# aditya-v-kallappa/FInCFlow

Measured on AMD Instinct MI355X. Metric: inverse images/sec (+ fwd+logdet ms/img in `forward`), 3x3 conv @64x64x96, higher is better.
Workload: dtype f32

## Files before the change

### fincflow_amd/csrc/finc_abi.hip

```cpp
#include "finc_common.h"

#include <stdlib.h>
#include <string.h>

#include <atomic>
#include <mutex>
#include <utility>
#include <vector>

namespace {

thread_local char g_hip_error[256] = "no error";

std::mutex g_table_mutex;
std::vector<std::pair<int, const void *>> g_attr_done;
constexpr int MAX_DEVICES = 64;
int *g_invariant_flag[MAX_DEVICES];
volatile unsigned *g_fault_host[MAX_DEVICES];
unsigned *g_fault_dev[MAX_DEVICES];
std::vector<std::pair<int, size_t>> g_debug_tokens;

std::atomic<bool> g_fault_armed_any{false};
std::vector<const char *> g_env_seen;

// ... 98 lines not shown

int finc_fault_gate(bool arm, hipStream_t st)
{
    if (!arm && !g_fault_armed_any.load(std::memory_order_acquire)) return FINC_OK;
    int dev = 0;
    FINC_HIP_TRY(hipGetDevice(&dev));
    if (dev < 0 || dev >= MAX_DEVICES) return FINC_ERR_BAD_DIMS;
    volatile unsigned *w = g_fault_host[dev];
    if (!w && arm) {
        hipStreamCaptureStatus cs = hipStreamCaptureStatusNone;
        if (hipStreamIsCapturing(st, &cs) != hipSuccess) { (void)hipGetLastError(); cs = hipStreamCaptureStatusNone; }
        if (cs == hipStreamCaptureStatusNone) {
            std::lock_guard<std::mutex> lk(g_table_mutex);
            if (!g_fault_host[dev]) {
                unsigned *h = nullptr, *d = nullptr;
                FINC_HIP_TRY(hipHostMalloc((void **)&h, sizeof(unsigned), hipHostMallocMapped));
                *h = 0;
                int e = FINC_OK;
                if (hipError_t he = hipHostGetDevicePointer((void **)&d, h, 0); he != hipSuccess) { finc_set_hip_error(he); e = FINC_ERR_LAUNCH; }
                if (!e) e = finc_mfma_arm_fault_word(d);
                if (e) { (void)hipHostFree(h); return e; }
                g_fault_dev[dev] = d;
                g_fault_host[dev] = h;
                g_fault_armed_any.store(true, std::memory_order_release);
            }
            w = g_fault_host[dev];
        }
    }
    if (w && *w != 0) {
        strncpy(g_hip_error, "a helper-wave wait of an earlier launch on this device gave up: its output is not valid (finc_clear_fault() resets)",
                sizeof(g_hip_error) - 1);
        return FINC_ERR_LAUNCH;
    }
    return FINC_OK;
}

template <typename T>
static int canonicalize(const T *w_stored, T *w_canon, int G, int Cq, int KH, int KW, unsigned orient, finc_stream_t stream)
{
    if (!w_stored || !w_canon) return FINC_ERR_NULL_POINTER;
    if (int e = check_shape(1, G, Cq, 1, 1, KH, KW)) return e;
    if (w_stored == w_canon) return FINC_ERR_BAD_DIMS;
    const int total = G * Cq * Cq * KH * KW;
    int blocks = (total + 255) / 256;
    if (blocks > 1024) blocks = 1024;
    hipLaunchKernelGGL(canonicalize_kernel<T>, dim3(blocks), dim3(256), 0, (hipStream_t)stream, w_stored, w_canon, G,
                       Cq, KH, KW, orient);
    FINC_CHECK_LAUNCH();
    return FINC_OK;
}

extern "C" {

int finc_version(void) { return 105; }

unsigned finc_build_flags(void)
{
    return FINC_BUILD_FLAGS | finc_build_flags_mfma() | finc_build_flags_split() | finc_build_flags_chain() | finc_build_flags_f64() | finc_build_flags_conv() | finc_build_flags_gradw() | finc_build_flags_wino4m() |
           finc_build_flags_mix() | finc_build_flags_generic() | finc_build_flags_wino() | finc_build_flags_big() | finc_build_flags_probe() | finc_build_flags_wino5() | finc_build_flags_stream();
}

int finc_fault_pending(void)
{
    int dev = 0;
    if (hipGetDevice(&dev) != hipSuccess || dev < 0 || dev >= MAX_DEVICES) return 0;
    volatile unsigned *w = g_fault_host[dev];
    return (w && *w != 0) ? 1 : 0;
}

int finc_runtime_switches(char *h_buf, size_t n)
{
    std::lock_guard<std::mutex> lk(g_table_mutex);
    size_t used = 0;
    int count = 0;
    auto put = [&](const char *t) {
        const size_t l = strlen(t);
        if (h_buf && used + l + 2 < n) {
            if (used) h_buf[used++] = ',';
            memcpy(h_buf + used, t, l);
            used += l;
        }
        ++count;
    };
    for (const char *name : g_env_seen) put(name);
    if (finc_wino_form_override() != 0) put("forward_form_override");
    if (h_buf && n) h_buf[used < n ? used : n - 1] = 0;
    return count;
}

int finc_clear_fault(void)
{
    int dev = 0;
    FINC_HIP_TRY(hipGetDevice(&dev));
    if (dev < 0 || dev >= MAX_DEVICES) return FINC_ERR_BAD_DIMS;
    if (g_fault_host[dev]) *g_fault_host[dev] = 0;
    return FINC_OK;
}

const char *finc_status_string(int status)
{
    switch (status) {
    case FINC_OK: return "ok";
    case FINC_ERR_NULL_POINTER: return "null pointer argument";
    case FINC_ERR_BAD_DIMS: return "bad dimensions";
    case FINC_ERR_UNSUPPORTED: return "requested algorithm does not support this shape";
    case FINC_ERR_WORKSPACE: return "workspace missing or too small";
    case FINC_ERR_LAUNCH: return "HIP call failed";
// ... 511 lines not shown
```

### fincflow_amd/csrc/finc_mfma.hip

```cpp
#include "finc_common.h"
#include "finc_tile.h"

#include <stdlib.h>

#include <mutex>
#include <type_traits>
#include <utility>
#include <vector>

namespace {

typedef float v4f __attribute__((ext_vector_type(4)));
typedef unsigned v2u __attribute__((ext_vector_type(2)));
typedef unsigned v4u __attribute__((ext_vector_type(4)));

template <int CQP_, int KH_, int KW_, int NW_ = 1>
struct Cfg {
    static constexpr int CQP = CQP_, KH = KH_, KW = KW_, NW = NW_;
    static constexpr int MTB = CQP / 16;
    static constexpr int NSM = (CQP % 16) / 4;
    static constexpr int MT = MTB + NSM;
    static constexpr int NKZT = CQP / 4;
    static constexpr int NKDT = CQP / 4;
    static_assert(NW == 1 || (NKZT % NW == 0 && NKDT % NW == 0), "K-split must divide the k-steps and the output registers");
    static constexpr int NKZ = NKZT / NW;
    static constexpr int NKD = NKDT / NW;
    static constexpr int NK = NKD;
    static constexpr int NTAP = KH * KW;
    static constexpr int NFRAG = (NKZ + (NTAP - 1) * NKD) * MT;
    static constexpr int NFRAGT = (NKZT + (NTAP - 1) * NKDT) * MT;
    static constexpr int NPACK = NFRAGT + 8 * MT;
    static constexpr int ZSLOTS = 12, XSLOTS = 8;
    static constexpr int ZRING = NKZ * ZSLOTS * 64;
    static constexpr int XRING = NKD * XSLOTS * 64;
    static constexpr bool XALIAS = NW == 2;
    static constexpr bool PAIR = finc_pair_bank(CQP, KH, KW) && NW == 1;
    static constexpr int NPAIR = 2 * NKDT;
    static constexpr int XCH = (NW > 1 && !XALIAS) ? NW * NW * NKD * 64 : 0;
};

__host__ __device__ inline int chan_d(int MTB, int j, int q)
{
    if (j < 4 * MTB) return 16 * (j >> 2) + 4 * q + (j & 3);
    return 16 * MTB + 4 * (j - 4 * MTB) + q;
}

template <int N>
__device__ inline float row_shr(float old, float src)
{
    return __builtin_bit_cast(float, __builtin_amdgcn_update_dpp(__builtin_bit_cast(int, old),
                                                                 __builtin_bit_cast(int, src), 0x110 + N, 0xf, 0xf,
                                                                 false));
}

template <int A>
struct ShiftOp {
    template <int NK>
    static __device__ inline void apply(float (&dst)[NK], const float (&fifo)[NK], const float (&src)[NK])
    {
#pragma unroll
        for (int j = 0; j < NK; ++j) dst[j] = row_shr<A>(fifo[j], src[j]);
    }
};

template <class C>
__device__ inline void pack_d(const v4f (&acc)[C::MT], float (&xpk)[C::NKDT])
{
#pragma unroll
    for (int mt = 0; mt < C::MTB; ++mt) {
        xpk[4 * mt + 0] = acc[mt].x;
        xpk[4 * mt + 1] = acc[mt].y;
        xpk[4 * mt + 2] = acc[mt].z;
        xpk[4 * mt + 3] = acc[mt].w;
    }
#pragma unroll
    for (int sb = 0; sb < C::NSM; ++sb) xpk[4 * C::MTB + sb] = finc_block_reduce(acc[C::MTB + sb]);
}

template <int KH, int KW>
struct BTaps {
    static constexpr int count()
    {
        int n = 0;
        for (int a = 0; a < KH; ++a)
            for (int b = 0; b < KW; ++b) n += (a + b >= 2);
        return n;
    }
    static constexpr int a_of(int i)
    {
        for (int a = 0; a < KH; ++a)
            for (int b = 0; b < KW; ++b)
                if (a + b >= 2 && i-- == 0) return a;
        return 0;
    }
    static constexpr int b_of(int i)
    {
        for (int a = 0; a < KH; ++a)
            for (int b = 0; b < KW; ++b)
// ... 74 lines not shown
        __builtin_amdgcn_make_buffer_rsrc((void *)(in + (size_t)bg_in * CQ * HW), 0, (int)slab_bytes, 0x00020000);
    const __amdgpu_buffer_rsrc_t rout =
        __builtin_amdgcn_make_buffer_rsrc((void *)(out + (size_t)bg_out * CQ * HW), 0, (int)slab_bytes, 0x00020000);
    const int D = W - P + 1;
    const int fifo_n = D * SS;
    const int wave_lds = C::ZRING + C::XRING + fifo_n + SS + 64;
    float *const lds_p = lds + prob * (C::XCH + NW * wave_lds);
    float *xch = lds_p;
    float *zring = lds_p + C::XCH + wv * wave_lds;
    float *xring = zring + C::ZRING;
    auto zcell = [](int qq, int rr) {
        const int lo = ((rr >> 2) ^ ((0x3200 >> (4 * (rr & 3))) & 3)) | ((qq & 1) << 2);
        return lo | (((rr & 3) | ((qq >> 1) << 2)) << 3);
    };
    float *fifo = xring + C::XRING;
    const int trash = fifo_n + lane;
    const unsigned flag_a = (unsigned)(uintptr_t)(lds + 4 * wave_lds + 4 * prob);
    auto flag_set = [flag_a](auto word_c, int v) {
        constexpr int WORD = decltype(word_c)::value;
        (void)flag_a;
#ifdef FINC_HLP_INJECT_TIMEOUT
        if (WORD == 1 && v >= 8) return;
#endif
        if constexpr (HLP) asm volatile("ds_write_b32 %0, %1 offset:%2" ::"v"(flag_a), "v"(v), "n"(4 * WORD) : "memory");
    };
    auto flag_peek = [flag_a](auto word_c, int &reg) {
        constexpr int WORD = decltype(word_c)::value;
        (void)flag_a;
        if constexpr (HLP) asm volatile("ds_read_b32 %0, %1 offset:%2" : "=v"(reg) : "v"(flag_a), "n"(4 * WORD) : "memory");
    };
    auto flag_wait = [flag_a](auto word_c, int target) {
        constexpr int WORD = decltype(word_c)::value;
#ifndef FINC_HLP_NOWAIT
#define FINC_HLP_NOWAIT 0
#endif
        if constexpr (HLP && !((FINC_HLP_NOWAIT >> WORD) & 1)) {
            int budget = 1 << FINC_HLP_BUDGET_LOG2;
            for (; budget > 0; --budget) {
                int v;
                asm volatile("ds_read_b32 %0, %1 offset:%2\n\ts_waitcnt lgkmcnt(0)" : "=v"(v) : "v"(flag_a), "n"(4 * WORD) : "memory");
                if (__builtin_amdgcn_readfirstlane(v) >= target) break;
                __builtin_amdgcn_s_sleep(2);
            }
            if (budget == 0 && (threadIdx.x & 63) == 0) {
                atomicAdd(&finc_hlp_timeouts, 1u);
                if (finc_fault_word) __hip_atomic_store(finc_fault_word, 1u, __ATOMIC_RELAXED, __HIP_MEMORY_SCOPE_SYSTEM);
            }
        }
    };

    constexpr int NSMALL = (NFRAG / MT) * C::NSM, NSR = (NSMALL + 3) / 4;
    float af[NFRAG];
    float afs[NSR > 0 ? NSR : 1];
    float afp[C::PAIR ? C::NPAIR : 1];
    static_assert(!C::PAIR || ((NKZ * C::NSM) % 4 == 0 && (NK * C::NSM) % 4 == 0),
                  "a packed block register must not straddle a paired and an unpaired tap");
    auto small_paired = [](int sfr) {
        const int tapi = sfr < NKZ * C::NSM ? 0 : 1 + (sfr - NKZ * C::NSM) / (NK * (C::NSM > 0 ? C::NSM : 1));
        return C::PAIR && tapi >= 1 && tapi <= 4;
    };
    if (!helper) {
        const float *pk = packed + (size_t)g * C::NPACK * 64 + lane;
        auto gindex = [&](int f) {
            if (f < NKZ * MT) return (wv * NKZ + f / MT) * MT + f % MT;
            const int ff = f - NKZ * MT;
            return C::NKZT * MT + ((ff / (MT * NKD)) * C::NKDT + wv * NKD + (ff / MT) % NKD) * MT + ff % MT;
        };
#pragma unroll
        for (int f = 0; f < NFRAG; ++f) {
            if (f % MT >= C::MTB) continue;
            if (ZPRE && f < NKZ * MT) { af[f] = 0.f; continue; }
            if (NW == 1 && f < NKZ * MT && finc_zterm_is_zero(C::MTB, f / MT, f % MT)) { af[f] = 0.f; continue; }
            af[f] = pk[gindex(f) * 64];
        }
        const int quad = (lane & 15) >> 2;
#pragma unroll
        for (int r = 0; r < NSR; ++r) {
            if (small_paired(4 * r)) { afs[r] = 0.f; continue; }
            int gi = 0;
#pragma unroll
            for (int a = 3; a >= 0; --a) {
                const int sfr = 4 * r + a < NSMALL ? 4 * r + a : NSMALL - 1;
                constexpr int NSMD = C::NSM > 0 ? C::NSM : 1;
                const int f = (sfr / NSMD) * MT + C::MTB + sfr % NSMD;
                const int ga = gindex(f);
                gi = (a == 3 || quad == a) ? ga : gi;
            }
            afs[r] = pk[gi * 64];
        }
#pragma unroll
        for (int f = 0; f < NFRAG; ++f) {
            if (f % MT >= C::MTB) continue;
            if (ZPRE && f < NKZ * MT) continue;
            if (NW == 1 && f < NKZ * MT && finc_zterm_is_zero(C::MTB, f / MT, f % MT)) continue;
            asm volatile("" : "+a"(af[f]));
        }
#pragma unroll
        for (int r = 0; r < NSR; ++r) {
            if (small_paired(4 * r)) continue;
            asm volatile("" : "+a"(afs[r]));
        }
        if constexpr (C::PAIR) {
            const float *pp = packed + finc_pair_offset(G, C::NPACK, C::NPAIR, g, 0) + lane;
#pragma unroll
            for (int f = 0; f < C::NPAIR; ++f) afp[f] = pp[f * 64];
#pragma unroll
            for (int f = 0; f < C::NPAIR; ++f) asm volatile("" : "+a"(afp[f]));
        }
    }
    auto mma = [&](v4f &acc_, int f, float b) {
        const int mt = f % MT;
        if (mt < C::MTB) acc_ = __builtin_amdgcn_mfma_f32_16x16x4f32(af[f], b, acc_, 0, 0, 0);
        else {
            const int sfr = (f / MT) * C::NSM + (mt - C::MTB);
            finc_mma_small(acc_, afs[sfr >> 2], b, sfr & 3);
        }
    };
    v4f bias[MT];
    {
        const float *pb = packed + ((size_t)g * C::NPACK + C::NFRAGT + (wv == 0 ? 0 : 4 * MT)) * 64 + lane;
#pragma unroll
        for (int mt = 0; mt < MT; ++mt)
            bias[mt] = (v4f){pb[(4 * mt + 0) * 64], pb[(4 * mt + 1) * 64], pb[(4 * mt + 2) * 64], pb[(4 * mt + 3) * 64]};
    }
    for (int i = lane; i < fifo_n + SS + 64; i += 64) fifo[i] = 0.f;

    const int fl4 = -((p + 3) >> 2);
    const int k0 = fw ? 3 : 0, k1 = fw ? 2 : 1, k2 = fw ? 1 : 2, k3 = fw ? 0 : 3;
    const unsigned lane_t = 4u * (unsigned)q * HW * 4u, lane_b = (unsigned)q * HW * 4u;
    unsigned cmask[NKD];
#pragma unroll
    for (int j = 0; j < NKD; ++j) cmask[j] = chan_d(C::MTB, wv * NKD + j, q) < CQ ? 0u : OFF_BAD_CHANNEL;
    const unsigned zlast = (4 * (wv * NKZ + NKZ - 1) + q) < CQ ? 0u : OFF_BAD_CHANNEL;
    unsigned zpad[NW > 1 ? NKZ : 1];
    if constexpr (NW > 1) {
#pragma unroll
        for (int j = 0; j < NKZ; ++j) zpad[j] = (4 * (wv * NKZ + j) + q) < CQ ? 0u : OFF_BAD_CHANNEL;
    }
    auto zmark = [&](int j) { return NW > 1 ? zpad[j] : (j == NKZ - 1 ? zlast : 0u); };
    const int rowstep = (fh ? -P : P) * W * 4;
    const int dirw = fw ? -1 : 1;

    constexpr unsigned long long PARTNER = 0xCBAFED8943276501ull;
    const int cls = ((p + 3) >> 2) & 1;
    const int part = (int)((PARTNER >> (4 * p)) & 15);
    int srvrow[2], srvhalf[2];
#pragma unroll
    for (int wp = 0; wp < 2; ++wp) {
        const bool own = cls == wp || p >= P;
        srvrow[wp] = own ? p : part;
        srvhalf[wp] = own ? 0 : 1;
    }
    int lcolS[2], lrowS[2], loffS[2], lslotS[2], ldst[2];
    int scolS[2], srowS[2], soffS[2];
#pragma unroll
    for (int wp = 0; wp < 2; ++wp) {
        const int R = srvrow[wp], h = srvhalf[wp];
        const int f = -((R + 3) >> 2);
        lcolS[wp] = 4 * ((wp ? -3 : -4) + 4 + f);
        lrowS[wp] = R;
// ... 439 lines not shown
                s64_part(IC<0>{}, IC<VMS>{}, w, IC<1>{});
                flag_wait(IC<0>{}, w);
                sec_sread(IC<1>{}, w + 1);
                s64_part(IC<0>{}, IC<VMS>{}, 0, IC<2>{});
                sec_swrite(IC<1>{}, 0, NKD);
                flag_wait(IC<3>{}, w + 1);
                s64_part(IC<1>{}, IC<VMS>{}, w + 1, IC<1>{});
                flag_wait(IC<0>{}, w + 1);
                sec_sread(IC<0>{}, w + 2);
                s64_part(IC<1>{}, IC<VMS>{}, 0, IC<2>{});
                sec_swrite(IC<0>{}, 0, NKD);
            }
            return;
        }
    }

    if constexpr (HLP) {
    } else if constexpr (SEC) {
        sec_event(IC<0>{});
        sec_event(IC<1>{});
        sec_event(IC<0>{});
        s64_event(IC<0>{}, IC<0>{});
        s64_event(IC<1>{}, IC<0>{});
        s64_event(IC<0>{}, IC<0>{});
    } else {
        io_issue(0, NKZ, true);
        io_land();
        io_issue(0, NKZ, true);
    }

    int nslot = ((-3 - p) % 12 + 12) % 12;
    const float *zrd = zring + (nslot >> 2) * 256 + 4 * zcell(q, p) + (fw ? 3 - (nslot & 3) : (nslot & 3));
    int zstep[4];
#pragma unroll
    for (int ph = 0; ph < 4; ++ph) zstep[ph] = (((ph + 2 - p) & 3) == 0) ? 256 - 3 * dirw : dirw;
    int tp1 = -3;
    int tm = -3;
    int xwin = 256 + lane;
    int win = 0;
    int peek_b = -1, peek_b2 = 0;

    {
        constexpr int FZ = 0;
        constexpr int FT = NKZ * MT;
        using BT = BTaps<KH, KW>;
        constexpr int NCH = BT::count();
        v4f acc[MT];
#pragma unroll
        for (int mt = 0; mt < MT; ++mt) acc[mt] = (v4f){0.f, 0.f, 0.f, 0.f};
        float zqc[C::NSM > 0 ? C::NSM : 1], zqn[C::NSM > 0 ? C::NSM : 1];
#pragma unroll
        for (int sb = 0; sb < (C::NSM > 0 ? C::NSM : 1); ++sb) zqc[sb] = zqn[sb] = 0.f;
        v4f accp = (v4f){0.f, 0.f, 0.f, 0.f};

        auto phase_a = [&](auto pha_c, int j0, int j1) {
            constexpr int PHA = decltype(pha_c)::value;
#pragma unroll
            for (int j = j0; j < j1; ++j)
#pragma unroll
                for (int mt = 0; mt < (C::PAIR ? C::MTB : MT); ++mt) {
                    if constexpr (KW > 1)
                        mma(acc[mt], FT + ((0 * KW + 1 - 1) * NK + j) * MT + mt, ROT ? Q[0][(PHA + 3) & 3][j] : R[0][1][j]);
                    if constexpr (KH > 1)
                        mma(acc[mt], FT + ((1 * KW + 0 - 1) * NK + j) * MT + mt, ROT ? Q[1][(PHA + 3) & 3][j] : R[1][0][j]);
                }
            if constexpr (C::PAIR) {
#pragma unroll
                for (int j = j0; j < j1; ++j) {
                    accp = __builtin_amdgcn_mfma_f32_16x16x4f32(afp[j], Q[0][(PHA + 3) & 3][j], accp, 0, 0, 0);
                    accp = __builtin_amdgcn_mfma_f32_16x16x4f32(afp[NK + j], Q[1][(PHA + 3) & 3][j], accp, 0, 0, 0);
                }
            }
        };

#ifdef FINC_STAMP
        unsigned stamp_acc[40];
#pragma unroll
        for (int i = 0; i < 40; ++i) stamp_acc[i] = 0u;
        unsigned long long stamp_prev = 0;
        bool stamp_on = false;
#endif
        auto step = [&](auto ph_c, auto wp_c) {
            constexpr int PH = decltype(ph_c)::value;
            FINC_STAMP_AT(9);
            const bool any_wrap = tm >= 0 && tm < P;
            const bool any_idle = tp1 < P - 1;
            float zraw[NKZ], zv[NKZ], xpk[NKD];
            float xown[NKD];
            v4f accn[MT];
            if constexpr (HLP && PH == 0) {
                asm volatile("s_waitcnt lgkmcnt(0)" ::: "memory");
                if (__builtin_expect(__builtin_amdgcn_readfirstlane(peek_b) < win, 0)) { FINC_COLD(); FINC_HLP_LATE(0); flag_wait(IC<1>{}, win); }
            }
            if constexpr (HLP && PH == 1) flag_peek(IC<2>{}, peek_b2);
            if constexpr (C::PAIR) {
                float rs[C::NSM];
#pragma unroll
                for (int sb = 0; sb < C::NSM; ++sb) {
                    rs[sb] = finc_block_reduce(acc[C::MTB + sb]);
                    if constexpr (ZPRE) rs[sb] += zqc[sb];
                }
                const float c0 = accp.z, c1 = accp.w;
                accp = (v4f){c0 + rs[0], c1 + rs[1], 0.f, 0.f};
            }

#pragma unroll
            for (int j = 0; j < NKZ; ++j) zraw[j] = FINC_ABLATE >= 3 ? af[j] : zrd[j * C::ZSLOTS * 64];
            if constexpr (!ROT) {
#pragma unroll
                for (int a = 0; a < KH; ++a) {
#pragma unroll
                    for (int b = KW - 1; b >= 1; --b) {
                        if (a + b >= 2) {
#pragma unroll
                            for (int j = 0; j < NK; ++j) R[a][b][j] = R[a][b - 1][j];
                        }
                    }
                    if (a >= 2) {
#pragma unroll
                        for (int j = 0; j < NK; ++j) R[a][0][j] = DL[a][a - 2][j];
                    }
                }
                if (__builtin_expect(any_wrap, 0)) {
                    FINC_COLD();
                    const bool wrapn = p == tm;
#pragma unroll
                    for (int a = 0; a < KH; ++a)
#pragma unroll
                        for (int b = 1; b < KW; ++b) {
                            if (a + b >= 2) {
#pragma unroll
                                for (int j = 0; j < NK; ++j) R[a][b][j] = wrapn ? 0.f : R[a][b][j];
                            }
                        }
                }
            }
            phase_a(ph_c, 0, NK / 2);
            if constexpr (HLP && PH == 3) flag_set(IC<3>{}, win + 1);
            FINC_SB();
#pragma unroll
            for (int j = 0; j < NKZ; ++j) zv[j] = zraw[j];
            if (__builtin_expect(any_idle, 0)) {
                FINC_COLD();
                const bool started = p <= tp1;
#pragma unroll
                for (int j = 0; j < NKZ; ++j) zv[j] = started ? zv[j] : 0.f;
            }
            phase_a(ph_c, NK / 2, NK);
            FINC_STAMP_AT(0);
            if constexpr (ROT) {
                if (__builtin_expect(any_wrap, 0)) {
                    FINC_COLD();
                    const bool wrapn = p == tm;
#pragma unroll
                    for (int a = 0; a < KH; ++a)
#pragma unroll
                        for (int b = 1; b < KW; ++b) {
                            if (a + b >= 2) {
#pragma unroll
                                for (int j = 0; j < NK; ++j)
                                    Q[a][(PH + 9 - a - b) & 3][j] = wrapn ? 0.f : Q[a][(PH + 9 - a - b) & 3][j];
                            }
                        }
                }
            }
            FINC_SB();
            if constexpr (ZPRE) {
#pragma unroll
                for (int mt = 0; mt < C::MTB; ++mt) accn[mt] = (v4f){zv[4 * mt], zv[4 * mt + 1], zv[4 * mt + 2], zv[4 * mt + 3]};
#pragma unroll
                for (int sb = 0; sb < C::NSM; ++sb) {
                    accn[C::MTB + sb] = (v4f){0.f, 0.f, 0.f, 0.f};
                    zqn[sb] = zv[4 * C::MTB + sb];
                }
            } else if (__builtin_expect(any_idle, 0)) {
                FINC_COLD();
                const bool started = p <= tp1;
#pragma unroll
                for (int mt = 0; mt < MT; ++mt) {
                    const float b0 = bias[mt].x, b1 = bias[mt].y, b2 = bias[mt].z, b3 = bias[mt].w;
                    accn[mt] = (v4f){started ? b0 : 0.f, started ? b1 : 0.f, started ? b2 : 0.f, started ? b3 : 0.f};
                    mma(accn[mt], FZ + mt, zv[0]);
                }
            } else {
#pragma unroll
                for (int mt = 0; mt < MT; ++mt) {
                    accn[mt] = bias[mt];
                    mma(accn[mt], FZ + mt, zv[0]);
                }
            }
#pragma unroll
            for (int j = 1; j < NKZ; ++j)
#pragma unroll
                for (int mt = 0; mt < MT; ++mt) {
                    if (ZPRE) continue;
                    if (NW == 1 && finc_zterm_is_zero(C::MTB, j, mt)) continue;
                    mma(accn[mt], FZ + j * MT + mt, zv[j]);
                }
            FINC_STAMP_AT(1);
            if constexpr (NW > 1) {
                float vv[C::NKDT];
                pack_d<C>(acc, vv);
#pragma unroll
                for (int d = 0; d < C::NKDT; ++d) {
                    const int dst = d / NKD;
                    if (dst != wv) {
                        if constexpr (C::XALIAS)
                            (lds_p + dst * wave_lds + C::ZRING)[(d % NKD) * C::XSLOTS * 64 + PH * 64 + xwin] = vv[d];
                        else
                            xch[((dst * NW + wv) * NKD + d % NKD) * 64 + lane] = vv[d];
                    }
                    else xown[d % NKD] = vv[d];
                }
                FINC_SB();
                __syncthreads();
            }
            FINC_SB();

            auto post1 = [&]() {
                if constexpr (FINC_ABLATE >= 2 && NW == 1) {
                    pack_d<C>(acc, xpk);
#pragma unroll
                    for (int j = 0; j < NKD; ++j) asm volatile("" ::"v"(xpk[j]));
                    return;
                }
                if constexpr (C::PAIR) {
#pragma unroll
                    for (int mt = 0; mt < C::MTB; ++mt) {
                        xpk[4 * mt + 0] = acc[mt].x;
                        xpk[4 * mt + 1] = acc[mt].y;
                        xpk[4 * mt + 2] = acc[mt].z;
                        xpk[4 * mt + 3] = acc[mt].w;
                    }
                    xpk[4 * C::MTB + 0] = accp.x;
                    xpk[4 * C::MTB + 1] = accp.y;
                    if (__builtin_expect(any_wrap, 0)) {
                        FINC_COLD();
                        const bool wrapn = p == tm;
                        const float c0 = accp.z, c1 = accp.w;
                        accp.z = wrapn ? 0.f : c0;
                        accp.w = wrapn ? 0.f : c1;
                    }
                } else if constexpr (NW == 1) {
                    pack_d<C>(acc, xpk);
                    if constexpr (ZPRE) {
#pragma unroll
                        for (int sb = 0; sb < C::NSM; ++sb) xpk[4 * C::MTB + sb] += zqc[sb];
                    }
                } else {
#pragma unroll
                    for (int j = 0; j < NKD; ++j) {
                        float sum = xown[j];
#pragma unroll
                        for (int src = 0; src < NW; ++src)
                            if (src != wv)
                                sum += C::XALIAS ? xring[j * C::XSLOTS * 64 + PH * 64 + xwin]
                                                 : xch[((wv * NW + src) * NKD + j) * 64 + lane];
                        xpk[j] = sum;
                    }
                }
#pragma unroll
                for (int j = 0; j < NKD; ++j) xring[j * C::XSLOTS * 64 + PH * 64 + xwin] = xpk[j];
                if constexpr (KH > 1) {
                    fifo_push(xpk);
                    fifo_pop_all();
                }
                if constexpr (KW > 1) {
                    if (__builtin_expect(any_wrap, 0)) {
                        FINC_COLD();
                        const bool wrapn = p == tm;
#pragma unroll
                        for (int j = 0; j < NK; ++j) (ROT ? Q[0][PH][j] : R[0][1][j]) = wrapn ? 0.f : xpk[j];
                    } else {
#pragma unroll
                        for (int j = 0; j < NK; ++j) (ROT ? Q[0][PH][j] : R[0][1][j]) = xpk[j];
                    }
                }
            };
            auto post2 = [&]() { if constexpr (FINC_ABLATE < 2) shift_all(xpk, ph_c); };

            auto chunk = [&](auto ci_c) {
                constexpr int CI = decltype(ci_c)::value;
                constexpr int a = BT::a_of(CI), b = BT::b_of(CI);
#pragma unroll
                for (int j = 0; j < NK; ++j)
#pragma unroll
                    for (int mt = 0; mt < ((C::PAIR && a + b == 2 && a < 2) ? C::MTB : MT); ++mt)
                        mma(accn[mt], FT + ((a * KW + b - 1) * NK + j) * MT + mt, ROT ? Q[a][(PH + 9 - a - b) & 3][j] : R[a][b][j]);
                if constexpr (CI == 0) {
                    if constexpr (HLP && PH == 1) {
                        asm volatile("s_waitcnt lgkmcnt(0)" ::: "memory");
                        if (__builtin_expect(__builtin_amdgcn_readfirstlane(peek_b2) < win + 1, 0)) { FINC_COLD(); FINC_HLP_LATE(1); flag_wait(IC<2>{}, win + 1); }
                    }
                    post1();
                    if constexpr (HLP && PH == 3) flag_set(IC<0>{}, win + 1);
                }
                if constexpr (!HLP && CI == (NCH > 1 ? 1 : 0)) io_phase(ph_c, wp_c);
                if constexpr (CI == (NCH > 2 ? 2 : NCH - 1)) {
                    post2();
                    if constexpr (HLP && PH == 3) flag_peek(IC<1>{}, peek_b);
                }
                FINC_SB();
                if constexpr (CI < 6) FINC_STAMP_AT(2 + CI);
            };
            if constexpr (NCH == 0) {
                post1();
                io_phase(ph_c, wp_c);
                post2();
                FINC_SB();
            } else {
                [&]<int... I>(std::integer_sequence<int, I...>) { (chunk(IC<I>{}), ...); }
                (std::make_integer_sequence<int, NCH>{});
            }
#pragma unroll
            for (int mt = 0; mt < MT; ++mt) acc[mt] = accn[mt];
            if constexpr (ZPRE) {
#pragma unroll
                for (int sb = 0; sb < C::NSM; ++sb) zqc[sb] = zqn[sb];
            }
            if constexpr (NW > 1) __syncthreads();
            ++tp1;
            ++tm; if (tm == W) tm = 0;
            ++nslot; zrd += zstep[PH];
            if (nslot == 12) { nslot = 0; zrd -= 12 * 64; }
            if constexpr (PH == 3) { xwin ^= 256; ++win; }
            fifo_advance();
            FINC_STAMP_AT(8);
        };

        if constexpr (HLP) {
        } else if constexpr (SEC) {
            sec_sread(IC<1>{});
            sec_swrite(IC<1>{}, 0, NKD);
            sec_event(IC<1>{});
            s64_event(IC<1>{}, IC<0>{});
        } else {
            io_sread();
            io_swrite(0, NKD);
            io_land();
            io_issue(0, NKZ, true);
        }
// ... 112 lines not shown
        }
        packed[((size_t)g * npack + f) * 64 + lane] = (float)v;
    }
    for (int e = threadIdx.x; e < npair * 64; e += blockDim.x) {
        const int lane = e & 63, f = e >> 6;
        int row, j, q, a, b;
        finc_pair_elem(MTB, NKD, f, lane, &row, &j, &q, &a, &b);
        const int col = chan_d(MTB, j, q);
        double v = 0.0;
        if (row < Cq && col < Cq) {
            const int widx = (KH - 1 - a) * KW + (KW - 1 - b);
            for (int k = 0; k <= row; ++k) v -= Linv[row * Cq + k] * (double)wg[((size_t)k * Cq + col) * KK + widx];
        }
        packed[finc_pair_offset(gridDim.x, npack, npair, g, f) + lane] = (float)v;
    }
    for (int e = threadIdx.x; e < 8 * MT * 64; e += blockDim.x) {
        const int lane = e & 63, f = e >> 6;
        const int q = lane >> 4, mt = (f % (4 * MT)) >> 2, r = f & 3;
        const int row = mt < MTB ? 16 * mt + 4 * q + r : (q == 0 ? 16 * MTB + 4 * (mt - MTB) + r : Cq);
        double v = 0.0;
        if (f < 4 * MT && shift && row < Cq)
            for (int k = 0; k <= row; ++k) v += Linv[row * Cq + k] * (double)shift[g * Cq + k];
        packed[((size_t)g * npack + nfrag + f) * 64 + lane] = (float)v;
    }
}

typedef void (*wave_fn)(const float *, const float *, float *, int, int, int, int, int, int, unsigned);

struct Inst {
    int cqp, kh, kw;
    wave_fn fn;
    wave_fn fn_sec;
    wave_fn fn_s64;
    wave_fn fn_hlp;
    wave_fn fn_zpre;
    int nkz, nkd, nk, mt, nfrag, mtb;
    int nw, wnkz, wnkd;
    int npw;
    int max_problems;
};

template <int CQP, int KH, int KW, int NW = 1, int NPW = 1, int MAXP = 0>
constexpr Inst make_inst()
{
    using C = Cfg<CQP, KH, KW, NW>;
    constexpr int zskip = [] {
        int n = 0;
        for (int j = 0; j < C::NKZ; ++j)
            for (int mt = 0; mt < C::MTB; ++mt) n += finc_zterm_is_zero(C::MTB, j, mt) ? 1 : 0;
        return n;
    }();
    constexpr bool one = NW == 1 && NPW == 1;
    constexpr int pinned = (C::NFRAG / C::MT) * C::MTB - zskip + ((C::NFRAG / C::MT) * C::NSM + 3) / 4;
    static_assert(!C::PAIR || C::NPAIR == C::NK * C::NSM, "paired fragments must replace as many packed block registers");
    constexpr int mode = !one ? 0 : (pinned + 8 * C::NKZ + 8 * C::NKD <= 256) ? 3 : (pinned + 8 * C::NKD <= 256) ? 1 : 0;
    wave_fn f64 = nullptr, fhl = nullptr, fzp = nullptr;
    if constexpr (mode != 0) f64 = finc_wave_kernel<CQP, KH, KW, true, NW, NPW, mode>;
#ifndef FINC_HLP_MODE
#define FINC_HLP_MODE 1
#endif
    constexpr bool hlp_fits = 16 * C::NKZ + 4 * C::NKD <= 124 && 12 * C::NKD + 48 <= 124 && pinned <= 124 && (KH - 1 + KW) < 6;
    if constexpr (mode == 3 && FINC_HLP_MODE && hlp_fits) {
        fhl = finc_wave_kernel<CQP, KH, KW, true, NW, NPW, 3, 1>;
        fzp = finc_wave_kernel<CQP, KH, KW, true, NW, NPW, 3, 1, true>;
    }
    return Inst{CQP, KH, KW, finc_wave_kernel<CQP, KH, KW, false, NW, NPW>, finc_wave_kernel<CQP, KH, KW, true, NW, NPW>, f64, fhl, fzp,
                C::NKZT, C::NKDT, C::NK, C::MT, C::NFRAGT, C::MTB, NW, C::NKZ, C::NKD, NPW, MAXP};
}

#ifdef FINC_ONLY_C3
const Inst g_insts[] = {make_inst<24, 3, 3, 2, 2, 512>(), make_inst<24, 3, 3>(), make_inst<12, 3, 3>()};
#else
const Inst g_insts[] = {
    make_inst<4, 3, 3>(),  make_inst<8, 3, 3>(),  make_inst<12, 3, 3>(), make_inst<16, 3, 3>(),
    make_inst<20, 3, 3>(),
    make_inst<24, 3, 3, 2, 2, 512>(), make_inst<24, 3, 3>(), make_inst<28, 3, 3>(),
    make_inst<32, 3, 3, 2, 2>(), make_inst<32, 3, 3>(),
    make_inst<40, 3, 3, 2, 2>(), make_inst<40, 3, 3, 2>(), make_inst<48, 3, 3, 4>(), make_inst<64, 3, 3, 4>(),
    make_inst<4, 2, 2>(),  make_inst<8, 2, 2>(),  make_inst<12, 2, 2>(), make_inst<16, 2, 2>(), make_inst<24, 2, 2>(),
    make_inst<32, 2, 2, 2, 2>(), make_inst<32, 2, 2>(),
    make_inst<4, 5, 5>(),  make_inst<8, 5, 5>(),  make_inst<12, 5, 5>(), make_inst<16, 5, 5>(),
    make_inst<24, 5, 5, 2>(), make_inst<32, 5, 5, 4>(), make_inst<48, 5, 5, 4>(),
    make_inst<4, 3, 5>(),  make_inst<8, 3, 5>(),  make_inst<16, 3, 5>(),
    make_inst<4, 2, 3>(),  make_inst<8, 2, 3>(),  make_inst<16, 2, 3>(),
};
#endif

size_t lds_bytes(const Inst &i, int W, int P);

bool finc_no_hlp()
{
    static const bool off = [] { const char *e = finc_env("FINC_NO_HLP"); return e && e[0] == '1'; }();
    return off;
}

bool finc_no_s64()
{
    static const bool off = [] { const char *e = finc_env("FINC_NO_S64"); return e && e[0] == '1'; }();
    return off;
}

int padded_cq(int Cq, int KH, int KW)
{
    int best = 0;
    for (const Inst &i : g_insts)
        if (i.cqp >= Cq && i.kh == KH && i.kw == KW && (best == 0 || i.cqp < best)) best = i.cqp;
    if (best && best - Cq > 3) {
// ... 40 lines not shown
{
    const size_t D = (size_t)(W - P + 1);
    const size_t ss = (size_t)i.nk * 4 * (i.kh - 1);
    const size_t per_wave = (size_t)i.wnkz * 12 * 64 + (size_t)i.wnkd * 8 * 64 + D * ss + ss + 64;
    const size_t xch = i.nw > 2 ? (size_t)i.nw * i.nw * i.wnkd * 64 : 0;
    return sizeof(float) * (size_t)i.npw * (xch + (size_t)i.nw * per_wave);
}

}

#ifdef FINC_STAMP
extern "C" int finc_debug_stamps(unsigned long long *host_out, int n)
{
    return (int)hipMemcpyFromSymbol(host_out, HIP_SYMBOL(finc_stamp_buf), sizeof(unsigned long long) * (size_t)n);
}
#endif

int finc_mfma_arm_fault_word(unsigned *device_ptr_to_host_word)
{
    FINC_HIP_TRY(hipMemcpyToSymbol(HIP_SYMBOL(finc_fault_word), &device_ptr_to_host_word, sizeof(device_ptr_to_host_word)));
    return FINC_OK;
}

int finc_mfma_hlp_timeouts(unsigned *count)
{
    FINC_HIP_TRY(hipMemcpyFromSymbol(count, HIP_SYMBOL(finc_hlp_timeouts), sizeof(unsigned)));
    return FINC_OK;
}

static bool stream_bank(int Cq, int KH, int KW)
{
    return !finc_big_bank(Cq, KH, KW) && padded_cq(Cq, KH, KW) == 0 && finc_stream_bank_ok(Cq, KH, KW);
}

static const Inst *bank_inst(int Cq, int KH, int KW)
{
    const int cqp = padded_cq(Cq, KH, KW);
    for (const Inst &i : g_insts)
        if (cqp && i.cqp == cqp && i.kh == KH && i.kw == KW) return &i;
    return nullptr;
}
static const Inst *borrowed_inst(int Cq, int KH, int KW)
{
    const int b = borrowed_cqp(padded_cq(Cq, KH, KW), KH, KW);
    if (b)
        for (const Inst &k : g_insts)
            if (k.cqp == b && k.kh == KH && k.kw == KW && k.nw == 2 && k.npw == 2) return &k;
    return nullptr;
}
static int pair_frags(const Inst *i)
{
    if (!finc_pair_bank(i->cqp, i->kh, i->kw)) return 0;
    for (const Inst &k : g_insts)
        if (k.cqp == i->cqp && k.kh == i->kh && k.kw == i->kw && k.nw == 1) return 2 * i->nkd;
    return 0;
}
static size_t bank_bytes(const Inst *i, int G) { return i ? (size_t)(i->nfrag + 8 * i->mt + pair_frags(i)) * 64 * sizeof(float) * (size_t)G : 0; }
static size_t wave_bank_bytes(int G, int Cq, int KH, int KW)
{
    return bank_bytes(bank_inst(Cq, KH, KW), G) + bank_bytes(borrowed_inst(Cq, KH, KW), G);
}

enum InvForm {
    INV_NONE,
    INV_TABLE,
    INV_SPLIT,
    INV_BIG,
    INV_WIDE,
    INV_STREAM,
};

struct InvPlan {
    InvForm form = INV_NONE;
    const Inst *inst = nullptr;
    int io = 0;
    wave_fn fn = nullptr;
    size_t lds = 0;
    int grid = 0, block = 0;
    size_t bank_offset = 0;
    int tail_images = 0;
    bool zpre = false;
    bool affine = false;
    bool align16 = true;
    FincSplitPlan split{};
};

static InvForm inverse_form(int Cq, int H, int W, int KH, int KW)
{
    if (finc_big_bank(Cq, KH, KW)) return finc_big_supported(Cq, H, W, KH, KW) ? INV_BIG : INV_NONE;
    if (stream_bank(Cq, KH, KW)) return finc_stream_supported(Cq, H, W, KH, KW, true) ? INV_STREAM : INV_NONE;
    if (W % 4 != 0 || W < 4 || H < 1) return INV_NONE;
    const int P = W < 16 ? W : 16;
    if (P < KH - 1) return INV_NONE;
    if (!find_inst(padded_cq(Cq, KH, KW), KH, KW, -1, W))
        return finc_big_wide_bank(Cq, KH, KW) && finc_big_supported(Cq, H, W, KH, KW) ? INV_WIDE : INV_NONE;
    if ((size_t)Cq * H * W * 4 >= ((size_t)1 << 30)) return INV_NONE;
    return INV_TABLE;
}

static InvPlan inverse_plan(const FincShape &s)
{
    InvPlan p;
    p.form = inverse_form(s.Cq, s.H, s.W, s.KH, s.KW);
    if (p.form == INV_NONE) return p;
    p.affine = p.form != INV_BIG && p.form != INV_WIDE;
    if (p.form == INV_WIDE) p.bank_offset = wave_bank_bytes(s.G, s.Cq, s.KH, s.KW);
    if (p.form == INV_BIG || p.form == INV_WIDE) return p;
// ... 206 lines not shown
```

### fincflow_amd/csrc/finc_tile.h

```cpp
#pragma once
#include <stddef.h>

typedef float finc_v4f __attribute__((ext_vector_type(4)));
typedef unsigned finc_v2u __attribute__((ext_vector_type(2)));

template <int MTB>
__device__ inline void finc_mma(finc_v4f &acc, int mt, float a, float b)
{
    if (mt < MTB) acc = __builtin_amdgcn_mfma_f32_16x16x4f32(a, b, acc, 0, 0, 0);
    else acc = __builtin_amdgcn_mfma_f32_4x4x1f32(a, b, acc, 0, 0, 0);
}

__device__ inline void finc_mma_small(finc_v4f &acc, float a4, float b, int abid)
{
    switch (abid & 3) {
    case 0: acc = __builtin_amdgcn_mfma_f32_4x4x1f32(a4, b, acc, 2, 0, 0); break;
    case 1: acc = __builtin_amdgcn_mfma_f32_4x4x1f32(a4, b, acc, 2, 1, 0); break;
    case 2: acc = __builtin_amdgcn_mfma_f32_4x4x1f32(a4, b, acc, 2, 2, 0); break;
    default: acc = __builtin_amdgcn_mfma_f32_4x4x1f32(a4, b, acc, 2, 3, 0); break;
    }
}

__device__ inline float finc_block_reduce(const finc_v4f &acc)
{
    const float r0 = acc.x, r1 = acc.y, r2 = acc.z, r3 = acc.w;
    const finc_v2u a = __builtin_amdgcn_permlane32_swap(__builtin_bit_cast(unsigned, r0), __builtin_bit_cast(unsigned, r2),
                                                        false, false);
    const finc_v2u b = __builtin_amdgcn_permlane32_swap(__builtin_bit_cast(unsigned, r1), __builtin_bit_cast(unsigned, r3),
                                                        false, false);
    const unsigned a0 = a.x, a1 = a.y, b0 = b.x, b1 = b.y;
    const float s02 = __builtin_bit_cast(float, a0) + __builtin_bit_cast(float, a1);
    const float s13 = __builtin_bit_cast(float, b0) + __builtin_bit_cast(float, b1);
    const finc_v2u c = __builtin_amdgcn_permlane16_swap(__builtin_bit_cast(unsigned, s02), __builtin_bit_cast(unsigned, s13),
                                                        false, false);
    const unsigned c0 = c.x, c1 = c.y;
    return __builtin_bit_cast(float, c0) + __builtin_bit_cast(float, c1);
}

__host__ __device__ constexpr bool finc_zterm_is_zero(int MTB, int j, int mt)
{
    return mt < MTB ? 4 * j > 16 * mt + 15 : 4 * j > 16 * MTB + 4 * (mt - MTB) + 3;
}

__host__ __device__ inline int finc_tile_row(int MTB, int mt, int i)
{
    return mt < MTB ? 16 * mt + i : 16 * MTB + 4 * (mt - MTB) + (i & 3);
}

__host__ __device__ constexpr bool finc_pair_bank(int cqp, int KH, int KW) { return KH == 3 && KW == 3 && cqp > 16 && cqp % 16 == 8; }
__host__ __device__ inline int finc_pair_row(int MTB, int i, int *partner)
{
    const int qq = i >> 2, r = i & 3;
    *partner = r >> 1;
    return 16 * MTB + 4 * (r & 1) + qq;
}
__host__ __device__ inline void finc_pair_elem(int MTB, int NKD, int f, int lane, int *row, int *j, int *q, int *a, int *b)
{
    int partner;
    const int pr = f / NKD;
    *row = finc_pair_row(MTB, lane & 15, &partner);
    *j = f % NKD;
    *q = lane >> 4;
    *a = pr == 0 ? 0 : 1;
    *b = (pr == 0 ? 1 : 0) + partner;
}
__host__ __device__ inline size_t finc_pair_offset(int G, int npack, int npair, int g, int f)
{
    return ((size_t)G * npack + (size_t)g * npair + f) * 64;
}
```

Before: 635,100.

## Extend paired-tap MFMA packing to the bottom kernel row in helper kernels

Adds a second stage of paired-fragment packing so that taps 6 and 7 (third kernel row) of the 3x3 wave kernel for odd-16 channel counts are computed with one 16x16x4 MFMA per k-step instead of separate small 4x4 block MFMAs. The carried column values go into a separate register pair and a new accumulator. The wrap test becomes a scalar sign-bit check. The new path is active only in helper (HLP) instantiations. It grows the paired weight bank from two to three fragments per k-step, which adds register and memory pressure and changes the packed layout every consumer must agree on.

```diff
diff --git a/fincflow_amd/csrc/finc_abi.hip b/fincflow_amd/csrc/finc_abi.hip
--- a/fincflow_amd/csrc/finc_abi.hip
+++ b/fincflow_amd/csrc/finc_abi.hip
@@ -174,7 +174,7 @@
 
 extern "C" {
 
-int finc_version(void) { return 105; }
+int finc_version(void) { return 106; }
 
 unsigned finc_build_flags(void)
 {
diff --git a/fincflow_amd/csrc/finc_mfma.hip b/fincflow_amd/csrc/finc_mfma.hip
--- a/fincflow_amd/csrc/finc_mfma.hip
+++ b/fincflow_amd/csrc/finc_mfma.hip
@@ -35,7 +35,8 @@
     static constexpr int XRING = NKD * XSLOTS * 64;
     static constexpr bool XALIAS = NW == 2;
     static constexpr bool PAIR = finc_pair_bank(CQP, KH, KW) && NW == 1;
-    static constexpr int NPAIR = 2 * NKDT;
+    static constexpr int NPAIR = 3 * NKDT;
+    static constexpr int NPAIR1 = 2 * NKDT;
     static constexpr int XCH = (NW > 1 && !XALIAS) ? NW * NW * NKD * 64 : 0;
 };
 
@@ -44,6 +45,9 @@
     if (j < 4 * MTB) return 16 * (j >> 2) + 4 * q + (j & 3);
     return 16 * MTB + 4 * (j - 4 * MTB) + q;
 }
+
+template <class C>
+__host__ __device__ constexpr bool finc_pair2_form(bool hlp) { return C::PAIR && hlp; }
 
 template <int N>
 __device__ inline float row_shr(float old, float src)
@@ -224,12 +228,14 @@
     constexpr int NSMALL = (NFRAG / MT) * C::NSM, NSR = (NSMALL + 3) / 4;
     float af[NFRAG];
     float afs[NSR > 0 ? NSR : 1];
-    float afp[C::PAIR ? C::NPAIR : 1];
+    constexpr bool PAIR2 = finc_pair2_form<C>(HLP);
+    constexpr int NPAIRF = PAIR2 ? C::NPAIR : C::NPAIR1;
+    float afp[C::PAIR ? NPAIRF : 1];
     static_assert(!C::PAIR || ((NKZ * C::NSM) % 4 == 0 && (NK * C::NSM) % 4 == 0),
                   "a packed block register must not straddle a paired and an unpaired tap");
     auto small_paired = [](int sfr) {
         const int tapi = sfr < NKZ * C::NSM ? 0 : 1 + (sfr - NKZ * C::NSM) / (NK * (C::NSM > 0 ? C::NSM : 1));
-        return C::PAIR && tapi >= 1 && tapi <= 4;
+        return C::PAIR && ((tapi >= 1 && tapi <= 4) || (PAIR2 && (tapi == 6 || tapi == 7)));
     };
     if (!helper) {
         const float *pk = packed + (size_t)g * C::NPACK * 64 + lane;
@@ -275,9 +281,9 @@
         if constexpr (C::PAIR) {
             const float *pp = packed + finc_pair_offset(G, C::NPACK, C::NPAIR, g, 0) + lane;
 #pragma unroll
-            for (int f = 0; f < C::NPAIR; ++f) afp[f] = pp[f * 64];
-#pragma unroll
-            for (int f = 0; f < C::NPAIR; ++f) asm volatile("" : "+a"(afp[f]));
+            for (int f = 0; f < NPAIRF; ++f) afp[f] = pp[f * 64];
+#pragma unroll
+            for (int f = 0; f < NPAIRF; ++f) asm volatile("" : "+a"(afp[f]));
         }
     }
     auto mma = [&](v4f &acc_, int f, float b) {
@@ -823,6 +829,8 @@
 #pragma unroll
         for (int sb = 0; sb < (C::NSM > 0 ? C::NSM : 1); ++sb) zqc[sb] = zqn[sb] = 0.f;
         v4f accp = (v4f){0.f, 0.f, 0.f, 0.f};
+        v4f accq = (v4f){0.f, 0.f, 0.f, 0.f};
+        float cy[2] = {0.f, 0.f};
 
         auto phase_a = [&](auto pha_c, int j0, int j1) {
             constexpr int PHA = decltype(pha_c)::value;
@@ -854,7 +862,17 @@
         auto step = [&](auto ph_c, auto wp_c) {
             constexpr int PH = decltype(ph_c)::value;
             FINC_STAMP_AT(9);
-            const bool any_wrap = tm >= 0 && tm < P;
+            std::conditional_t<C::PAIR, int, bool> wrap_state;
+            if constexpr (C::PAIR) wrap_state = (tm - P) & ~tm;
+            else wrap_state = tm >= 0 && tm < P;
+            auto any_wrap = [&]() -> bool {
+                if constexpr (C::PAIR) {
+                    asm volatile("" : "+s"(wrap_state));
+                    return wrap_state < 0;
+                } else {
+                    return wrap_state;
+                }
+            };
             const bool any_idle = tp1 < P - 1;
             float zraw[NKZ], zv[NKZ], xpk[NKD];
             float xown[NKD];
@@ -871,8 +889,14 @@
                     rs[sb] = finc_block_reduce(acc[C::MTB + sb]);
                     if constexpr (ZPRE) rs[sb] += zqc[sb];
                 }
-                const float c0 = accp.z, c1 = accp.w;
-                accp = (v4f){c0 + rs[0], c1 + rs[1], 0.f, 0.f};
+                if constexpr (PAIR2) {
+                    accp = accq;
+                    accp.x += cy[0] + rs[0];
+                    accp.y += cy[1] + rs[1];
+                } else {
+                    const float c0 = accp.z, c1 = accp.w;
+                    accp = (v4f){c0 + rs[0], c1 + rs[1], 0.f, 0.f};
+                }
             }
 
 #pragma unroll
@@ -892,7 +916,7 @@
                         for (int j = 0; j < NK; ++j) R[a][0][j] = DL[a][a - 2][j];
                     }
                 }
-                if (__builtin_expect(any_wrap, 0)) {
+                if (__builtin_expect(any_wrap(), 0)) {
                     FINC_COLD();
                     const bool wrapn = p == tm;
 #pragma unroll
@@ -920,7 +944,7 @@
             phase_a(ph_c, NK / 2, NK);
             FINC_STAMP_AT(0);
             if constexpr (ROT) {
-                if (__builtin_expect(any_wrap, 0)) {
+                if (__builtin_expect(any_wrap(), 0)) {
                     FINC_COLD();
                     const bool wrapn = p == tm;
 #pragma unroll
@@ -1005,12 +1029,21 @@
                     }
                     xpk[4 * C::MTB + 0] = accp.x;
                     xpk[4 * C::MTB + 1] = accp.y;
-                    if (__builtin_expect(any_wrap, 0)) {
+                    if constexpr (PAIR2) {
+                        cy[0] = accp.z;
+                        cy[1] = accp.w;
+                    }
+                    if (__builtin_expect(any_wrap(), 0)) {
                         FINC_COLD();
                         const bool wrapn = p == tm;
                         const float c0 = accp.z, c1 = accp.w;
-                        accp.z = wrapn ? 0.f : c0;
-                        accp.w = wrapn ? 0.f : c1;
+                        if constexpr (PAIR2) {
+                            cy[0] = wrapn ? 0.f : c0;
+                            cy[1] = wrapn ? 0.f : c1;
+                        } else {
+                            accp.z = wrapn ? 0.f : c0;
+                            accp.w = wrapn ? 0.f : c1;
+                        }
                     }
                 } else if constexpr (NW == 1) {
                     pack_d<C>(acc, xpk);
@@ -1036,8 +1069,11 @@
                     fifo_push(xpk);
                     fifo_pop_all();
                 }
-                if constexpr (KW > 1) {
-                    if (__builtin_expect(any_wrap, 0)) {
+                if constexpr (C::PAIR) {
+#pragma unroll
+                    for (int j = 0; j < NK; ++j) Q[0][PH][j] = xpk[j];
+                } else if constexpr (KW > 1) {
+                    if (__builtin_expect(any_wrap(), 0)) {
                         FINC_COLD();
                         const bool wrapn = p == tm;
 #pragma unroll
@@ -1048,7 +1084,17 @@
                     }
                 }
             };
-            auto post2 = [&]() { if constexpr (FINC_ABLATE < 2) shift_all(xpk, ph_c); };
+            auto post2 = [&]() {
+                if constexpr (FINC_ABLATE < 2) shift_all(xpk, ph_c);
+                if constexpr (C::PAIR && FINC_ABLATE < 2) {
+                    if (__builtin_expect(any_wrap(), 0)) {
+                        FINC_COLD();
+                        const bool wrapn = p == tm;
+#pragma unroll
+                        for (int j = 0; j < NK; ++j) Q[0][PH][j] = wrapn ? 0.f : Q[0][PH][j];
+                    }
+                }
+            };
 
             auto chunk = [&](auto ci_c) {
                 constexpr int CI = decltype(ci_c)::value;
@@ -1056,8 +1102,13 @@
 #pragma unroll
                 for (int j = 0; j < NK; ++j)
 #pragma unroll
-                    for (int mt = 0; mt < ((C::PAIR && a + b == 2 && a < 2) ? C::MTB : MT); ++mt)
+                    for (int mt = 0; mt < ((C::PAIR && ((a + b == 2 && a < 2) || (PAIR2 && a == 2 && b < 2))) ? C::MTB : MT); ++mt)
                         mma(accn[mt], FT + ((a * KW + b - 1) * NK + j) * MT + mt, ROT ? Q[a][(PH + 9 - a - b) & 3][j] : R[a][b][j]);
+                if constexpr (PAIR2 && a == 2 && b == 0) {
+#pragma unroll
+                    for (int j = 0; j < NK; ++j)
+                        accq = __builtin_amdgcn_mfma_f32_16x16x4f32(afp[2 * NK + j], Q[2][(PH + 7) & 3][j], j == 0 ? (v4f){0.f, 0.f, 0.f, 0.f} : accq, 0, 0, 0);
+                }
                 if constexpr (CI == 0) {
                     if constexpr (HLP && PH == 1) {
                         asm volatile("s_waitcnt lgkmcnt(0)" ::: "memory");
@@ -1276,7 +1327,8 @@
     }();
     constexpr bool one = NW == 1 && NPW == 1;
     constexpr int pinned = (C::NFRAG / C::MT) * C::MTB - zskip + ((C::NFRAG / C::MT) * C::NSM + 3) / 4;
-    static_assert(!C::PAIR || C::NPAIR == C::NK * C::NSM, "paired fragments must replace as many packed block registers");
+    static_assert(!C::PAIR || (C::NPAIR1 == 4 * C::NK * C::NSM / 4 && C::NPAIR == 6 * C::NK * C::NSM / 4),
+                  "paired fragments must replace as many packed block registers (stage 1: four taps, stage 2: six)");
     constexpr int mode = !one ? 0 : (pinned + 8 * C::NKZ + 8 * C::NKD <= 256) ? 3 : (pinned + 8 * C::NKD <= 256) ? 1 : 0;
     wave_fn f64 = nullptr, fhl = nullptr, fzp = nullptr;
     if constexpr (mode != 0) f64 = finc_wave_kernel<CQP, KH, KW, true, NW, NPW, mode>;
@@ -1423,7 +1475,7 @@
 {
     if (!finc_pair_bank(i->cqp, i->kh, i->kw)) return 0;
     for (const Inst &k : g_insts)
-        if (k.cqp == i->cqp && k.kh == i->kh && k.kw == i->kw && k.nw == 1) return 2 * i->nkd;
+        if (k.cqp == i->cqp && k.kh == i->kh && k.kw == i->kw && k.nw == 1) return 3 * i->nkd;
     return 0;
 }
 static size_t bank_bytes(const Inst *i, int G) { return i ? (size_t)(i->nfrag + 8 * i->mt + pair_frags(i)) * 64 * sizeof(float) * (size_t)G : 0; }
diff --git a/fincflow_amd/csrc/finc_tile.h b/fincflow_amd/csrc/finc_tile.h
--- a/fincflow_amd/csrc/finc_tile.h
+++ b/fincflow_amd/csrc/finc_tile.h
@@ -61,7 +61,7 @@
     *row = finc_pair_row(MTB, lane & 15, &partner);
     *j = f % NKD;
     *q = lane >> 4;
-    *a = pr == 0 ? 0 : 1;
+    *a = pr;
     *b = (pr == 0 ? 1 : 0) + partner;
 }
 __host__ __device__ inline size_t finc_pair_offset(int G, int npack, int npair, int g, int f)
```

Measured after the change: 645,300, median of 6. +1.6%, better.
